# ashys2012/MDC-Net-Multimodal-Defect-Captioning-Network-For-Surface-Steel-Defects

Measured on NVIDIA B200. Metric: images/sec end-to-end encode+greedy decode, higher is better.
Workload: dtype bf16

## Files before the change

### mdc-net-multimodal-defect-captioning-network-for-surface-steel-defects_b200/csrc/attention_umma.cu

```cuda
#include "common.cuh"
#include <cuda.h>
#include <stdlib.h>

namespace {

constexpr int HD = 64;
constexpr int QROWS = 256;
constexpr int N_SOFTMAX_WARPS = 16;
constexpr int THREADS = 64 + N_SOFTMAX_WARPS * 32;

struct SmemLayout {
  int q_bytes, kv_bytes, buf_bytes;
};

__global__ void __launch_bounds__(THREADS, 1)
attn_umma_kernel(const __grid_constant__ CUtensorMap map_q, const __grid_constant__ CUtensorMap map_kv, bf16* __restrict__ out, int64_t ldo,
                 int n_items, int S, int H, int NK, float scale_log2e, long long* dbg) {
#ifdef MDC_DEVTOOLS
#define STAMP(i) do { if (dbg && blockIdx.x == 0 && n == 0) dbg[i] = clock64(); } while (0)
#else
#define STAMP(i) do { } while (0)
#endif
  extern __shared__ uint8_t smem_raw[];
  uint8_t* smem = (uint8_t*)(((uintptr_t)smem_raw + 1023) & ~(uintptr_t)1023);
  const int q_bytes = QROWS * 128, kv_bytes = NK * 128, buf_bytes = q_bytes + 2 * kv_bytes;
  uint64_t* bars = (uint64_t*)(smem + 2 * buf_bytes);
  uint64_t* full = bars; uint64_t* sfree = bars + 2; uint64_t* s_ready = bars + 4; uint64_t* p_ready = bars + 6; uint64_t* o_ready = bars + 8;
  uint64_t* t_free = bars + 10;
  uint32_t* tmem_ptr_smem = (uint32_t*)(bars + 12);
  float* xch = (float*)(bars + 16);
  const int warp = threadIdx.x >> 5, lane = threadIdx.x & 31;
  const int tiles = S > 128 ? 2 : 1;

  if (threadIdx.x == 0) {
    for (int i = 0; i < 2; ++i) {
      mbar_init(smem_u32(&full[i]), 1); mbar_init(smem_u32(&sfree[i]), 1); mbar_init(smem_u32(&s_ready[i]), 1);
      mbar_init(smem_u32(&p_ready[i]), N_SOFTMAX_WARPS * 32); mbar_init(smem_u32(&o_ready[i]), 1); mbar_init(smem_u32(&t_free[i]), N_SOFTMAX_WARPS * 32);
    }
    fence_mbarrier_init();
    prefetch_tmap(&map_q);
    prefetch_tmap(&map_kv);
  }
  if (warp == 0) {
    tmem_alloc<1>(smem_u32(tmem_ptr_smem), 512);
    tmem_relinquish<1>();
  }
  tc_fence_before();
  __syncthreads();
  tc_fence_after();
  const uint32_t tmem_base = *tmem_ptr_smem;
  const int D = H * HD;

  if (warp == 1) {
    if (lane == 0) {
      int n = 0;
      for (int item = blockIdx.x; item < n_items; item += gridDim.x, ++n) {
        const int buf = n & 1, strip = item / H, head = item % H;
        mbar_wait(smem_u32(&sfree[buf]), ((n >> 1) & 1) ^ 1);
        const uint32_t fb = smem_u32(&full[buf]);
        const uint32_t base = smem_u32(smem + buf * buf_bytes);
        STAMP(0);
        mbar_expect_tx(fb, (uint32_t)(3 * kv_bytes));
        tma_load_2d(&map_kv, fb, base, head * HD, strip * S);
        tma_load_2d(&map_kv, fb, base + q_bytes, D + head * HD, strip * S);
        tma_load_2d(&map_kv, fb, base + q_bytes + kv_bytes, 2 * D + head * HD, strip * S);
      }
    }
  } else if (warp == 0) {
    if (lane == 0) {
      const uint32_t idesc_qk = make_idesc(128, NK), idesc_pv = make_idesc(128, HD, false, true);
      int n = 0;
      for (int item = blockIdx.x; item < n_items; item += gridDim.x, ++n) {
        const int buf = n & 1;
        const uint32_t base = smem_u32(smem + buf * buf_bytes);
        mbar_wait(smem_u32(&full[buf]), (n >> 1) & 1);
        STAMP(1);
        tc_fence_after();
        const uint64_t kdesc = make_sw128_desc(base + q_bytes);
        for (int t = 0; t < tiles; ++t) {
          mbar_wait(smem_u32(&t_free[t]), (n & 1) ^ 1);
          tc_fence_after();
          const uint64_t qdesc = make_sw128_desc(base + t * 128 * 128);
#pragma unroll
          for (int k = 0; k < HD / 16; ++k) umma_ss(tmem_base + t * 256, qdesc + 2 * k, kdesc + 2 * k, idesc_qk, k != 0);
          umma_commit(smem_u32(&s_ready[t]));
          STAMP(2 + t);
        }
        const uint64_t vdesc = make_sw128_desc(base + q_bytes + kv_bytes);
        for (int t = 0; t < tiles; ++t) {
          mbar_wait(smem_u32(&p_ready[t]), n & 1);
          STAMP(4 + t);
          tc_fence_after();
          for (int k = 0; k < NK / 16; ++k)
            umma_ts(tmem_base + t * 256 + 128, tmem_base + t * 256 + 8 * k, vdesc + (uint64_t)(128 * k), idesc_pv, k != 0);
          umma_commit(smem_u32(&o_ready[t]));
          STAMP(6 + t);
        }
        umma_commit(smem_u32(&sfree[buf]));
      }
    }
  } else {
    const int sw = warp - 2, part = sw >> 2, row = 32 * (warp & 3) + lane;
    const int qc = NK / 4;
    const int nch = qc / 4;
    const uint32_t lane_addr = (uint32_t)(32 * (warp & 3)) << 16;
    int n = 0;
    for (int item = blockIdx.x; item < n_items; item += gridDim.x, ++n) {
      const int strip = item / H, head = item % H;
      float rsum[2] = {0.f, 0.f};
      for (int t = 0; t < tiles; ++t) {
        mbar_wait(smem_u32(&s_ready[t]), n & 1);
        if (threadIdx.x == 64) STAMP(10 + 8 * t);
        tc_fence_after();
        const uint32_t trow = tmem_base + lane_addr + t * 256;
        const bool live = __any_sync(0xffffffffu, t * 128 + row < S);
        float s[64];
        if (live) {
          uint32_t* sr = reinterpret_cast<uint32_t*>(s);
          const uint32_t tcol = trow + part * qc;
          if (nch >= 8) {
            tmem_ld32(tcol, sr);
            if (nch == 16) tmem_ld32(tcol + 32, sr + 32);
            else if (nch >= 12) {
              tmem_ld16(tcol + 32, sr + 32);
#pragma unroll
              for (int c = 12; c < 15; ++c) if (c < nch) tmem_ld4(tcol + 4 * c, sr + 4 * c);
            } else {
#pragma unroll
              for (int c = 8; c < 11; ++c) if (c < nch) tmem_ld4(tcol + 4 * c, sr + 4 * c);
            }
          } else if (nch >= 4) {
            tmem_ld16(tcol, sr);
#pragma unroll
            for (int c = 4; c < 7; ++c) if (c < nch) tmem_ld4(tcol + 4 * c, sr + 4 * c);
          } else {
#pragma unroll
            for (int c = 0; c < 3; ++c) if (c < nch) tmem_ld4(tcol + 4 * c, sr + 4 * c);
          }
          tmem_ld_wait();
        }
        if (threadIdx.x == 64) STAMP(11 + 8 * t);
        const int nvalid = min(max(S - part * qc, 0), qc);
        float m4[4] = {-INFINITY, -INFINITY, -INFINITY, -INFINITY};
        if (live) {
#pragma unroll
          for (int c = 0; c < 16; ++c)
            if (c < nch) {
              if (4 * c + 4 <= nvalid) {
#pragma unroll
                for (int j = 0; j < 4; ++j) m4[j] = fmaxf(m4[j], s[4 * c + j]);
              } else {
#pragma unroll
                for (int j = 0; j < 4; ++j) {
                  if (4 * c + j >= nvalid) s[4 * c + j] = -INFINITY;
                  m4[j] = fmaxf(m4[j], s[4 * c + j]);
                }
              }
            }
        }
        float mx = fmaxf(fmaxf(m4[0], m4[1]), fmaxf(m4[2], m4[3]));
        xch[part * 128 + row] = mx;
        bar_sync<128>(1 + (warp & 3));
        if (threadIdx.x == 64) STAMP(12 + 8 * t);
        mx = fmaxf(fmaxf(xch[row], xch[128 + row]), fmaxf(xch[256 + row], xch[384 + row]));
        const float nms = -mx * scale_log2e;
        float s4[4] = {0.f, 0.f, 0.f, 0.f};
        if (live) {
#pragma unroll
          for (int c = 0; c < 16; ++c)
            if (c < nch) {
              float p[4];
#pragma unroll
              for (int j = 0; j < 4; ++j) { p[j] = ex2_approx(fmaf(s[4 * c + j], scale_log2e, nms)); s4[j] += p[j]; }
              tmem_st2(trow + (part * qc) / 2 + 2 * c, pack_bf16x2(p[0], p[1]), pack_bf16x2(p[2], p[3]));
            }
        }
        const float sum = (s4[0] + s4[1]) + (s4[2] + s4[3]);
        rsum[t] = sum;
        xch[512 + t * 512 + part * 128 + row] = sum;
        if (threadIdx.x == 64) STAMP(13 + 8 * t);
        tmem_st_wait();
        if (threadIdx.x == 64) STAMP(14 + 8 * t);
        tc_fence_before();
        mbar_arrive(smem_u32(&p_ready[t]));
        bar_sync<128>(1 + (warp & 3));
      }
      for (int t = 0; t < tiles; ++t) {
        mbar_wait(smem_u32(&o_ready[t]), n & 1);
        if (threadIdx.x == 64) STAMP(26 + 2 * t);
        tc_fence_after();
        const uint32_t trow = tmem_base + lane_addr + t * 256 + 128;
        uint32_t o[16];
        tmem_ld16(trow + part * 16, o);
        tmem_ld_wait();
        tc_fence_before();
        mbar_arrive(smem_u32(&t_free[t]));
        const float* sx = xch + 512 + t * 512 + row;
        const float inv = 1.0f / ((sx[0] + sx[128]) + (sx[256] + sx[384]));
        const int q = t * 128 + row;
        if (q < S) {
          bf16* dst = out + ((int64_t)strip * S + q) * ldo + head * HD + part * 16;
#pragma unroll
          for (int j = 0; j < 16; j += 8) {
            uint4 v;
            v.x = pack_bf16x2(__uint_as_float(o[j]) * inv, __uint_as_float(o[j + 1]) * inv);
            v.y = pack_bf16x2(__uint_as_float(o[j + 2]) * inv, __uint_as_float(o[j + 3]) * inv);
            v.z = pack_bf16x2(__uint_as_float(o[j + 4]) * inv, __uint_as_float(o[j + 5]) * inv);
            v.w = pack_bf16x2(__uint_as_float(o[j + 6]) * inv, __uint_as_float(o[j + 7]) * inv);
            *reinterpret_cast<uint4*>(dst + j) = v;
          }
        }
      }
      if (threadIdx.x == 64) STAMP(30);
      bar_sync<128>(1 + (warp & 3));
    }
  }
  tc_fence_before();
  __syncthreads();
  if (warp == 0) {
    tc_fence_after();
    tmem_dealloc<1>(tmem_base, 512);
  }
}

}

int attn_umma_supported(int strip_len, int head_dim, int64_t ld, int64_t ldo) {
  return head_dim == HD && strip_len >= 16 && strip_len <= 256 && ld % 8 == 0 && ldo % 8 == 0;
}

int attn_umma_launch(mdc_ctx* ctx, const void* qkv, int64_t ld, void* out, int64_t ldo, int n_strips, int strip_len, int heads, float scale,
                     cudaStream_t s) {
  MDC_CHECK_ARG(((uintptr_t)qkv & 15) == 0 && ((uintptr_t)out & 15) == 0);
  const int S = strip_len, NK = ((S + 15) / 16) * 16;
  const int64_t rows = (int64_t)n_strips * S;
  CUtensorMap mq, mkv;
  MDC_TRY(mdc_make_tmap_2d(ctx, qkv, rows, 3 * heads * HD, ld, HD, NK, 3, &mkv));
  mq = mkv;
  const int buf_bytes = QROWS * 128 + 2 * NK * 128;
  const size_t smem = 2 * (size_t)buf_bytes + 1024 + 128 + 3 * 512 * 4;
  MDC_ENSURE_SMEM(attn_umma_kernel, smem);
  const int n_items = n_strips * heads;
  const int grid = n_items < ctx->sm_count ? n_items : ctx->sm_count;
  long long* dbg = nullptr;
#ifdef MDC_DEVTOOLS
  if (const char* e = getenv("MDC_ATTN_TRACE_PTR")) dbg = (long long*)strtoull(e, nullptr, 0);
#endif
  attn_umma_kernel<<<grid, THREADS, smem, s>>>(mq, mkv, (bf16*)out, ldo, n_items, S, heads, NK, scale * LOG2E, dbg);
  MDC_LAUNCH_CHECK(ctx);
  return 0;
}
```

Baseline: 13190.

## Split attention work into 128-row query tiles with dedicated epilogue warps

Attention work is now split per 128-row query tile instead of per (strip, head), so the grid covers more work units when S exceeds 128. The MMA warp issues QK for the next two tiles ahead, keeping both TMEM/smem slots busy. Four new epilogue warps handle the O readout, normalization and stores, so the softmax warps can move on to the next tile's scores. In exchange, K and V are reloaded once per query tile rather than once per item, the block gains 128 threads, and the mbarrier parity logic becomes more involved.

```diff
diff --git a/mdc-net-multimodal-defect-captioning-network-for-surface-steel-defects_b200/csrc/attention_umma.cu b/mdc-net-multimodal-defect-captioning-network-for-surface-steel-defects_b200/csrc/attention_umma.cu
--- a/mdc-net-multimodal-defect-captioning-network-for-surface-steel-defects_b200/csrc/attention_umma.cu
+++ b/mdc-net-multimodal-defect-captioning-network-for-surface-steel-defects_b200/csrc/attention_umma.cu
@@ -7,19 +7,17 @@
 constexpr int HD = 64;
 constexpr int QROWS = 256;
 constexpr int N_SOFTMAX_WARPS = 16;
-constexpr int THREADS = 64 + N_SOFTMAX_WARPS * 32;
-
-struct SmemLayout {
-  int q_bytes, kv_bytes, buf_bytes;
-};
+constexpr int N_EPI_WARPS = 4;
+constexpr int THREADS = 64 + (N_SOFTMAX_WARPS + N_EPI_WARPS) * 32;
+constexpr int XCH_FLOATS = 4 * 512;
 
 __global__ void __launch_bounds__(THREADS, 1)
 attn_umma_kernel(const __grid_constant__ CUtensorMap map_q, const __grid_constant__ CUtensorMap map_kv, bf16* __restrict__ out, int64_t ldo,
-                 int n_items, int S, int H, int NK, float scale_log2e, long long* dbg) {
+                 int n_work, int S, int H, int NK, float scale_log2e, long long* dbg) {
 #ifdef MDC_DEVTOOLS
-#define STAMP(i) do { if (dbg && blockIdx.x == 0 && n == 0) dbg[i] = clock64(); } while (0)
+#define STAMP(i, first) do { if (dbg && blockIdx.x == 0 && (first)) dbg[i] = clock64(); } while (0)
 #else
-#define STAMP(i) do { } while (0)
+#define STAMP(i, first) do { } while (0)
 #endif
   extern __shared__ uint8_t smem_raw[];
   uint8_t* smem = (uint8_t*)(((uintptr_t)smem_raw + 1023) & ~(uintptr_t)1023);
@@ -31,11 +29,12 @@
   float* xch = (float*)(bars + 16);
   const int warp = threadIdx.x >> 5, lane = threadIdx.x & 31;
   const int tiles = S > 128 ? 2 : 1;
+  const int n_tiles = (n_work - 1 - (int)blockIdx.x) / (int)gridDim.x + 1;
 
   if (threadIdx.x == 0) {
     for (int i = 0; i < 2; ++i) {
       mbar_init(smem_u32(&full[i]), 1); mbar_init(smem_u32(&sfree[i]), 1); mbar_init(smem_u32(&s_ready[i]), 1);
-      mbar_init(smem_u32(&p_ready[i]), N_SOFTMAX_WARPS * 32); mbar_init(smem_u32(&o_ready[i]), 1); mbar_init(smem_u32(&t_free[i]), N_SOFTMAX_WARPS * 32);
+      mbar_init(smem_u32(&p_ready[i]), N_SOFTMAX_WARPS * 32); mbar_init(smem_u32(&o_ready[i]), 1); mbar_init(smem_u32(&t_free[i]), N_EPI_WARPS * 32);
     }
     fence_mbarrier_init();
     prefetch_tmap(&map_q);
@@ -53,15 +52,15 @@
 
   if (warp == 1) {
     if (lane == 0) {
-      int n = 0;
-      for (int item = blockIdx.x; item < n_items; item += gridDim.x, ++n) {
-        const int buf = n & 1, strip = item / H, head = item % H;
-        mbar_wait(smem_u32(&sfree[buf]), ((n >> 1) & 1) ^ 1);
+      for (int j = 0; j < n_tiles; ++j) {
+        const int w = blockIdx.x + j * gridDim.x, item = w / tiles, t = w - item * tiles, strip = item / H, head = item % H;
+        const int buf = j & 1;
+        mbar_wait(smem_u32(&sfree[buf]), ((j >> 1) & 1) ^ 1);
         const uint32_t fb = smem_u32(&full[buf]);
         const uint32_t base = smem_u32(smem + buf * buf_bytes);
-        STAMP(0);
+        STAMP(j, j < 2);
         mbar_expect_tx(fb, (uint32_t)(3 * kv_bytes));
-        tma_load_2d(&map_kv, fb, base, head * HD, strip * S);
+        tma_load_2d(&map_kv, fb, base, head * HD, strip * S + t * 128);
         tma_load_2d(&map_kv, fb, base + q_bytes, D + head * HD, strip * S);
         tma_load_2d(&map_kv, fb, base + q_bytes + kv_bytes, 2 * D + head * HD, strip * S);
       }
@@ -69,150 +68,149 @@
   } else if (warp == 0) {
     if (lane == 0) {
       const uint32_t idesc_qk = make_idesc(128, NK), idesc_pv = make_idesc(128, HD, false, true);
-      int n = 0;
-      for (int item = blockIdx.x; item < n_items; item += gridDim.x, ++n) {
-        const int buf = n & 1;
-        const uint32_t base = smem_u32(smem + buf * buf_bytes);
-        mbar_wait(smem_u32(&full[buf]), (n >> 1) & 1);
-        STAMP(1);
+      auto issue_qk = [&](int j) {
+        const int r = j & 1;
+        const uint32_t base = smem_u32(smem + r * buf_bytes);
+        mbar_wait(smem_u32(&full[r]), (j >> 1) & 1);
+        STAMP(2 + j, j < 2);
+        mbar_wait(smem_u32(&t_free[r]), ((j >> 1) & 1) ^ 1);
         tc_fence_after();
-        const uint64_t kdesc = make_sw128_desc(base + q_bytes);
-        for (int t = 0; t < tiles; ++t) {
-          mbar_wait(smem_u32(&t_free[t]), (n & 1) ^ 1);
-          tc_fence_after();
-          const uint64_t qdesc = make_sw128_desc(base + t * 128 * 128);
-#pragma unroll
-          for (int k = 0; k < HD / 16; ++k) umma_ss(tmem_base + t * 256, qdesc + 2 * k, kdesc + 2 * k, idesc_qk, k != 0);
-          umma_commit(smem_u32(&s_ready[t]));
-          STAMP(2 + t);
-        }
-        const uint64_t vdesc = make_sw128_desc(base + q_bytes + kv_bytes);
-        for (int t = 0; t < tiles; ++t) {
-          mbar_wait(smem_u32(&p_ready[t]), n & 1);
-          STAMP(4 + t);
-          tc_fence_after();
-          for (int k = 0; k < NK / 16; ++k)
-            umma_ts(tmem_base + t * 256 + 128, tmem_base + t * 256 + 8 * k, vdesc + (uint64_t)(128 * k), idesc_pv, k != 0);
-          umma_commit(smem_u32(&o_ready[t]));
-          STAMP(6 + t);
-        }
-        umma_commit(smem_u32(&sfree[buf]));
-      }
-    }
-  } else {
+        const uint64_t qdesc = make_sw128_desc(base), kdesc = make_sw128_desc(base + q_bytes);
+#pragma unroll
+        for (int k = 0; k < HD / 16; ++k) umma_ss(tmem_base + r * 256, qdesc + 2 * k, kdesc + 2 * k, idesc_qk, k != 0);
+        umma_commit(smem_u32(&s_ready[r]));
+        STAMP(8 + 8 * j, j < 4);
+      };
+      issue_qk(0);
+      if (n_tiles > 1) issue_qk(1);
+      for (int j = 0; j < n_tiles; ++j) {
+        const int r = j & 1;
+        mbar_wait(smem_u32(&p_ready[r]), (j >> 1) & 1);
+        tc_fence_after();
+        const uint64_t vdesc = make_sw128_desc(smem_u32(smem + r * buf_bytes) + q_bytes + kv_bytes);
+        for (int k = 0; k < NK / 16; ++k)
+          umma_ts(tmem_base + r * 256 + 128, tmem_base + r * 256 + 8 * k, vdesc + (uint64_t)(128 * k), idesc_pv, k != 0);
+        umma_commit(smem_u32(&o_ready[r]));
+        STAMP(13 + 8 * j, j < 4);
+        umma_commit(smem_u32(&sfree[r]));
+        if (j + 2 < n_tiles) issue_qk(j + 2);
+      }
+    }
+  } else if (warp < 2 + N_SOFTMAX_WARPS) {
     const int sw = warp - 2, part = sw >> 2, row = 32 * (warp & 3) + lane;
     const int qc = NK / 4;
     const int nch = qc / 4;
     const uint32_t lane_addr = (uint32_t)(32 * (warp & 3)) << 16;
-    int n = 0;
-    for (int item = blockIdx.x; item < n_items; item += gridDim.x, ++n) {
-      const int strip = item / H, head = item % H;
-      float rsum[2] = {0.f, 0.f};
-      for (int t = 0; t < tiles; ++t) {
-        mbar_wait(smem_u32(&s_ready[t]), n & 1);
-        if (threadIdx.x == 64) STAMP(10 + 8 * t);
-        tc_fence_after();
-        const uint32_t trow = tmem_base + lane_addr + t * 256;
-        const bool live = __any_sync(0xffffffffu, t * 128 + row < S);
-        float s[64];
-        if (live) {
-          uint32_t* sr = reinterpret_cast<uint32_t*>(s);
-          const uint32_t tcol = trow + part * qc;
-          if (nch >= 8) {
-            tmem_ld32(tcol, sr);
-            if (nch == 16) tmem_ld32(tcol + 32, sr + 32);
-            else if (nch >= 12) {
-              tmem_ld16(tcol + 32, sr + 32);
-#pragma unroll
-              for (int c = 12; c < 15; ++c) if (c < nch) tmem_ld4(tcol + 4 * c, sr + 4 * c);
+    for (int j = 0; j < n_tiles; ++j) {
+      const int t = (blockIdx.x + j * gridDim.x) % tiles, r = j & 1;
+      mbar_wait(smem_u32(&s_ready[r]), (j >> 1) & 1);
+      if (threadIdx.x == 64) STAMP(9 + 8 * j, j < 4);
+      tc_fence_after();
+      const uint32_t trow = tmem_base + lane_addr + r * 256;
+      const bool live = __any_sync(0xffffffffu, t * 128 + row < S);
+      float s[64];
+      if (live) {
+        uint32_t* sr = reinterpret_cast<uint32_t*>(s);
+        const uint32_t tcol = trow + part * qc;
+        if (nch >= 8) {
+          tmem_ld32(tcol, sr);
+          if (nch == 16) tmem_ld32(tcol + 32, sr + 32);
+          else if (nch >= 12) {
+            tmem_ld16(tcol + 32, sr + 32);
+#pragma unroll
+            for (int c = 12; c < 15; ++c) if (c < nch) tmem_ld4(tcol + 4 * c, sr + 4 * c);
+          } else {
+#pragma unroll
+            for (int c = 8; c < 11; ++c) if (c < nch) tmem_ld4(tcol + 4 * c, sr + 4 * c);
+          }
+        } else if (nch >= 4) {
+          tmem_ld16(tcol, sr);
+#pragma unroll
+          for (int c = 4; c < 7; ++c) if (c < nch) tmem_ld4(tcol + 4 * c, sr + 4 * c);
+        } else {
+#pragma unroll
+          for (int c = 0; c < 3; ++c) if (c < nch) tmem_ld4(tcol + 4 * c, sr + 4 * c);
+        }
+        tmem_ld_wait();
+      }
+      if (threadIdx.x == 64) STAMP(10 + 8 * j, j < 4);
+      const int nvalid = min(max(S - part * qc, 0), qc);
+      float m4[4] = {-INFINITY, -INFINITY, -INFINITY, -INFINITY};
+      if (live) {
+#pragma unroll
+        for (int c = 0; c < 16; ++c)
+          if (c < nch) {
+            if (4 * c + 4 <= nvalid) {
+#pragma unroll
+              for (int e = 0; e < 4; ++e) m4[e] = fmaxf(m4[e], s[4 * c + e]);
             } else {
 #pragma unroll
-              for (int c = 8; c < 11; ++c) if (c < nch) tmem_ld4(tcol + 4 * c, sr + 4 * c);
-            }
-          } else if (nch >= 4) {
-            tmem_ld16(tcol, sr);
-#pragma unroll
-            for (int c = 4; c < 7; ++c) if (c < nch) tmem_ld4(tcol + 4 * c, sr + 4 * c);
-          } else {
-#pragma unroll
-            for (int c = 0; c < 3; ++c) if (c < nch) tmem_ld4(tcol + 4 * c, sr + 4 * c);
-          }
-          tmem_ld_wait();
-        }
-        if (threadIdx.x == 64) STAMP(11 + 8 * t);
-        const int nvalid = min(max(S - part * qc, 0), qc);
-        float m4[4] = {-INFINITY, -INFINITY, -INFINITY, -INFINITY};
-        if (live) {
-#pragma unroll
-          for (int c = 0; c < 16; ++c)
-            if (c < nch) {
-              if (4 * c + 4 <= nvalid) {
-#pragma unroll
-                for (int j = 0; j < 4; ++j) m4[j] = fmaxf(m4[j], s[4 * c + j]);
-              } else {
-#pragma unroll
-                for (int j = 0; j < 4; ++j) {
-                  if (4 * c + j >= nvalid) s[4 * c + j] = -INFINITY;
-                  m4[j] = fmaxf(m4[j], s[4 * c + j]);
-                }
+              for (int e = 0; e < 4; ++e) {
+                if (4 * c + e >= nvalid) s[4 * c + e] = -INFINITY;
+                m4[e] = fmaxf(m4[e], s[4 * c + e]);
               }
             }
+          }
+      }
+      float* xm = xch + r * 512;
+      float mx = fmaxf(fmaxf(m4[0], m4[1]), fmaxf(m4[2], m4[3]));
+      xm[part * 128 + row] = mx;
+      bar_sync<128>(1 + (warp & 3));
+      if (threadIdx.x == 64) STAMP(11 + 8 * j, j < 4);
+      mx = fmaxf(fmaxf(xm[row], xm[128 + row]), fmaxf(xm[256 + row], xm[384 + row]));
+      const float nms = -mx * scale_log2e;
+      float s4[4] = {0.f, 0.f, 0.f, 0.f};
+      if (live) {
+#pragma unroll
+        for (int c = 0; c < 16; ++c)
+          if (c < nch) {
+            float p[4];
+#pragma unroll
+            for (int e = 0; e < 4; ++e) { p[e] = ex2_approx(fmaf(s[4 * c + e], scale_log2e, nms)); s4[e] += p[e]; }
+            tmem_st2(trow + (part * qc) / 2 + 2 * c, pack_bf16x2(p[0], p[1]), pack_bf16x2(p[2], p[3]));
+          }
+      }
+      xch[1024 + r * 512 + part * 128 + row] = (s4[0] + s4[1]) + (s4[2] + s4[3]);
+      tmem_st_wait();
+      if (threadIdx.x == 64) STAMP(12 + 8 * j, j < 4);
+      tc_fence_before();
+      mbar_arrive(smem_u32(&p_ready[r]));
+    }
+  } else {
+    const int row = 32 * (warp & 3) + lane;
+    const uint32_t lane_addr = (uint32_t)(32 * (warp & 3)) << 16;
+    for (int j = 0; j < n_tiles; ++j) {
+      const int w = blockIdx.x + j * gridDim.x, item = w / tiles, t = w - item * tiles, r = j & 1;
+      const int strip = item / H, head = item % H;
+      mbar_wait(smem_u32(&p_ready[r]), (j >> 1) & 1);
+      const float* sx = xch + 1024 + r * 512 + row;
+      const float inv = 1.0f / ((sx[0] + sx[128]) + (sx[256] + sx[384]));
+      mbar_wait(smem_u32(&o_ready[r]), (j >> 1) & 1);
+      if (threadIdx.x == 64 + 32 * N_SOFTMAX_WARPS) STAMP(14 + 8 * j, j < 4);
+      tc_fence_after();
+      const int q = t * 128 + row;
+      uint32_t o[64];
+      if (__any_sync(0xffffffffu, q < S)) {
+        const uint32_t tcol = tmem_base + lane_addr + r * 256 + 128;
+        tmem_ld32(tcol, o);
+        tmem_ld32(tcol + 32, o + 32);
+        tmem_ld_wait();
+      }
+      tc_fence_before();
+      mbar_arrive(smem_u32(&t_free[r]));
+      if (threadIdx.x == 64 + 32 * N_SOFTMAX_WARPS) STAMP(15 + 8 * j, j < 4);
+      if (q < S) {
+        bf16* dst = out + ((int64_t)strip * S + q) * ldo + head * HD;
+#pragma unroll
+        for (int c = 0; c < HD; c += 8) {
+          uint4 v;
+          v.x = pack_bf16x2(__uint_as_float(o[c]) * inv, __uint_as_float(o[c + 1]) * inv);
+          v.y = pack_bf16x2(__uint_as_float(o[c + 2]) * inv, __uint_as_float(o[c + 3]) * inv);
+          v.z = pack_bf16x2(__uint_as_float(o[c + 4]) * inv, __uint_as_float(o[c + 5]) * inv);
+          v.w = pack_bf16x2(__uint_as_float(o[c + 6]) * inv, __uint_as_float(o[c + 7]) * inv);
+          *reinterpret_cast<uint4*>(dst + c) = v;
         }
-        float mx = fmaxf(fmaxf(m4[0], m4[1]), fmaxf(m4[2], m4[3]));
-        xch[part * 128 + row] = mx;
-        bar_sync<128>(1 + (warp & 3));
-        if (threadIdx.x == 64) STAMP(12 + 8 * t);
-        mx = fmaxf(fmaxf(xch[row], xch[128 + row]), fmaxf(xch[256 + row], xch[384 + row]));
-        const float nms = -mx * scale_log2e;
-        float s4[4] = {0.f, 0.f, 0.f, 0.f};
-        if (live) {
-#pragma unroll
-          for (int c = 0; c < 16; ++c)
-            if (c < nch) {
-              float p[4];
-#pragma unroll
-              for (int j = 0; j < 4; ++j) { p[j] = ex2_approx(fmaf(s[4 * c + j], scale_log2e, nms)); s4[j] += p[j]; }
-              tmem_st2(trow + (part * qc) / 2 + 2 * c, pack_bf16x2(p[0], p[1]), pack_bf16x2(p[2], p[3]));
-            }
-        }
-        const float sum = (s4[0] + s4[1]) + (s4[2] + s4[3]);
-        rsum[t] = sum;
-        xch[512 + t * 512 + part * 128 + row] = sum;
-        if (threadIdx.x == 64) STAMP(13 + 8 * t);
-        tmem_st_wait();
-        if (threadIdx.x == 64) STAMP(14 + 8 * t);
-        tc_fence_before();
-        mbar_arrive(smem_u32(&p_ready[t]));
-        bar_sync<128>(1 + (warp & 3));
-      }
-      for (int t = 0; t < tiles; ++t) {
-        mbar_wait(smem_u32(&o_ready[t]), n & 1);
-        if (threadIdx.x == 64) STAMP(26 + 2 * t);
-        tc_fence_after();
-        const uint32_t trow = tmem_base + lane_addr + t * 256 + 128;
-        uint32_t o[16];
-        tmem_ld16(trow + part * 16, o);
-        tmem_ld_wait();
-        tc_fence_before();
-        mbar_arrive(smem_u32(&t_free[t]));
-        const float* sx = xch + 512 + t * 512 + row;
-        const float inv = 1.0f / ((sx[0] + sx[128]) + (sx[256] + sx[384]));
-        const int q = t * 128 + row;
-        if (q < S) {
-          bf16* dst = out + ((int64_t)strip * S + q) * ldo + head * HD + part * 16;
-#pragma unroll
-          for (int j = 0; j < 16; j += 8) {
-            uint4 v;
-            v.x = pack_bf16x2(__uint_as_float(o[j]) * inv, __uint_as_float(o[j + 1]) * inv);
-            v.y = pack_bf16x2(__uint_as_float(o[j + 2]) * inv, __uint_as_float(o[j + 3]) * inv);
-            v.z = pack_bf16x2(__uint_as_float(o[j + 4]) * inv, __uint_as_float(o[j + 5]) * inv);
-            v.w = pack_bf16x2(__uint_as_float(o[j + 6]) * inv, __uint_as_float(o[j + 7]) * inv);
-            *reinterpret_cast<uint4*>(dst + j) = v;
-          }
-        }
-      }
-      if (threadIdx.x == 64) STAMP(30);
-      bar_sync<128>(1 + (warp & 3));
+      }
     }
   }
   tc_fence_before();
@@ -238,15 +236,15 @@
   MDC_TRY(mdc_make_tmap_2d(ctx, qkv, rows, 3 * heads * HD, ld, HD, NK, 3, &mkv));
   mq = mkv;
   const int buf_bytes = QROWS * 128 + 2 * NK * 128;
-  const size_t smem = 2 * (size_t)buf_bytes + 1024 + 128 + 3 * 512 * 4;
+  const size_t smem = 2 * (size_t)buf_bytes + 1024 + 128 + XCH_FLOATS * 4;
   MDC_ENSURE_SMEM(attn_umma_kernel, smem);
-  const int n_items = n_strips * heads;
-  const int grid = n_items < ctx->sm_count ? n_items : ctx->sm_count;
+  const int n_work = n_strips * heads * (S > 128 ? 2 : 1);
+  const int grid = n_work < ctx->sm_count ? n_work : ctx->sm_count;
   long long* dbg = nullptr;
 #ifdef MDC_DEVTOOLS
   if (const char* e = getenv("MDC_ATTN_TRACE_PTR")) dbg = (long long*)strtoull(e, nullptr, 0);
 #endif
-  attn_umma_kernel<<<grid, THREADS, smem, s>>>(mq, mkv, (bf16*)out, ldo, n_items, S, heads, NK, scale * LOG2E, dbg);
+  attn_umma_kernel<<<grid, THREADS, smem, s>>>(mq, mkv, (bf16*)out, ldo, n_work, S, heads, NK, scale * LOG2E, dbg);
   MDC_LAUNCH_CHECK(ctx);
   return 0;
 }
```

Result: no change. 13290, median of 6 (+0.8%).
